# rongzhao-zhang/EfficientQ

Hardware: AMD Instinct MI355X
Metric: ptq_calibration_throughput (higher is better)
Workload: dtype i8xi8->i32 (exact) for the Gram systems and per-iteration loss convs of the layers with quantised input, f32/f64 elsewhere

## Files before the change

### efficientq_amd/_lib.py

```python
from __future__ import annotations

import ctypes as C
import os

import torch

_HERE = os.path.dirname(os.path.abspath(__file__))
LIB_PATH = os.path.join(_HERE, "libeffq_hip.so")

EFFQ_OK = 0
_ERR_NAMES = {1: "EFFQ_ERR_ARG", 2: "EFFQ_ERR_HIP", 3: "EFFQ_ERR_WORKSPACE", 4: "EFFQ_ERR_NO_DEVICE",
              5: "EFFQ_ERR_NOT_CONVERGED"}


class EffqError(RuntimeError):
    pass


class Geom(C.Structure):
    _fields_ = [(n, C.c_int32) for n in
                ("N", "C1", "C2", "D", "H", "W", "KD", "KH", "KW", "SD", "SH", "SW", "PD", "PH", "PW")]

    def out_dims(self):
        return ((self.D + 2 * self.PD - self.KD) // self.SD + 1,
# ... 40 lines not shown


class ProfRecord(C.Structure):
    _fields_ = [("kind", C.c_int32), ("iter", C.c_int32), ("loss_kind", C.c_int32), ("c2", C.c_int32), ("n", C.c_int32),
                ("geom", Geom), ("ms", C.c_float)]


SIGNATURES = {
    "effq_last_error": (C.c_char_p, []),
    "effq_version": (_I, []),
    "effq_device_count": (_I, [C.POINTER(C.c_int)]),
    "effq_quant_dequant_f32": (_I, [_P, _P, _F, _F, _I, _P, _P, _SZ, _P]),
    "effq_quant_dequant_f64path": (_I, [_P, _P, _D, _D, _I, _P, _P, _P, _SZ, _P]),
    "effq_reduce_ws_bytes": (_SZ, []),
    "effq_abs_sum_f64": (_I, [_P, _SZ, _P, _P, _P]),
    "effq_moments_f64": (_I, [_P, _SZ, _P, _P, _P]),
    "effq_alpha_stats_f64": (_I, [_P, _P, _D, _D, _I, _SZ, _P, _P, _P, _P]),
    "effq_fp_init": (_I, [_P, _P, _P]),
    "effq_fp_update": (_I, [_P, _D, _I, _P]),
    "effq_alpha_fixed_point": (_I, [_P, _SZ, _I, _D, _D, _D, _I, _I, _P, _P, _P]),
    "effq_fp_small_max": (_SZ, []),
    "effq_fixed_point_small": (_I, [_P, _P, _P, _SZ, _I, _D, _D, _D, _I, _P, _P]),
    "effq_fp_coop_max": (_SZ, []),
    "effq_fp_coop_set_spin_limit": (_I, [C.c_uint]),
    "effq_fixed_point_coop": (_I, [_P, _P, _P, _SZ, _I, _D, _D, _D, _I, _P, _P, _P]),
    "effq_fp_bucket_max": (_SZ, []),
    "effq_fp_bucket_ws_bytes": (_SZ, [_SZ]),
    "effq_fixed_point_bucket": (_I, [_P, _P, _P, _SZ, _I, _D, _D, _D, _I, _P, _P, _SZ, _P]),
    "effq_fp_bracket_ws_bytes": (_SZ, [_SZ]),
    "effq_fp_bracket_init": (_I, [_P, _P, _SZ, _I, _I, _P, _SZ, _P]),
    "effq_fp_bracket_run": (_I, [_P, _SZ, _I, _D, _D, _D, _I, _I, _P, _P, _P]),
    "effq_fp_bracket_stats": (_I, [_P, _SZ, _I, _D, _D, _P, _P, _P]),
    "effq_fp_bracket_update": (_I, [_SZ, _I, _D, _D, _D, _I, _P, _P, _P]),
    "effq_fp_traj_max": (_SZ, []),
    "effq_fp_traj_ws_bytes": (_SZ, [_SZ]),
    "effq_spd_inverse_prepare": (_I, [_P]),
    "effq_fp_traj_pred_bytes": (_SZ, []),
    "effq_fixed_point_traj": (_I, [_P, _P, _P, _SZ, _I, _D, _D, _D, _I, _P, _P, _P, _SZ, _P]),
    "effq_fixed_point_bucket_rec": (_I, [_P, _P, _P, _SZ, _I, _D, _D, _D, _I, _P, _P, _SZ, _P, _P]),
    "effq_fixed_point_coop_rec": (_I, [_P, _P, _P, _SZ, _I, _D, _D, _D, _I, _P, _P, _P, _P]),
    "effq_fp_check": (_I, [_P, _P, _P]),
    "effq_fp_channels_max_row": (_I, []),
    "effq_fixed_point_channels": (_I, [_P, _P, _P, _I, _I, _I, _D, _I, _P, _P, _P, _P]),
    "effq_fixed_point_channels_proj": (_I, [_P, _P, _P, _I, _I, _I, _D, _I, _P, _P, _P, _P, _F, _P, _P, _P, _I, _I, _D,
                                            _D, _P]),
    "effq_gram_packed_elems": (_SZ, [_I, _I]),
    "effq_gram_pack": (_I, [_P, _P, _I, _I, _P, _P]),
    "effq_gram_unpack": (_I, [_P, _I, _I, _P, _P, _P]),
    "effq_act_quant_backward": (_I, [_P, _P, _I, _P, _P, _P, _SZ, _P, _P]),
    "effq_att_classes_ws_bytes": (_SZ, []),
    "effq_att_classes": (_I, [_P, _LL, _P, _P, _P, C.POINTER(C.c_int32), _P, _P]),
    "effq_prof_enable": (_I, [_I]),
    "effq_prof_count": (_I, []),
    "effq_prof_read": (_I, [_I, C.POINTER(ProfRecord)]),
    "effq_admm_num_inverses": (_I, [_D, _D, _I, _I]),
    "effq_admm_run": (_I, [C.POINTER(AdmmRunArgs)]),
    "effq_admm_select_best": (_I, [_P, _I, _P, _P, _SZ, _SZ, _P, _P, _P, _P]),
    "effq_gram_ws_bytes": (_SZ, [_GP, _I]),
    "effq_gram_accum": (_I, [_P, _P, _P, _GP, _I, _P, _P, _I, _P, _SZ, _P]),
    "effq_gram_plan_query": (_I, [_GP, _I, _IP, _IP, _IP, _IP, _LLP, _IP, _IP]),
    "effq_gram_streamed": (_I, [_P, _P, _GP, _I]),
    "effq_gram_finish": (_I, [_GP, _I, _P, _P, _I, _P, _SZ, _P]),
    "effq_gram_i8_supported": (_I, [_GP, _I]),
    "effq_gram_i8_ws_bytes": (_SZ, [_GP, _I]),
    "effq_gram_accum_i8": (_I, [_P, _P, _GP, _I, _P, _I, _P, _P, _P, _I, _LL, _P, _P, _I, _P, _SZ, _P]),
    "effq_gram_accum_i8_unw": (_I, [_P, _P, _GP, _I, _P, _I, _P, _P, _P, _I, _LL, _P, _P, _I, _P, _P, _P, _SZ, _P]),
# ... 144 lines not shown
```

### efficientq_amd/csrc/fixed_point_bracket.hip

```cpp
#include <math.h>
#include "common.h"
#include "fp_level.h"

namespace effq {

constexpr int FBR_T = 256;
constexpr int FBR_MAXG = 1024;
constexpr int FBR_FT = 1024;
constexpr size_t FBR_MIN_PER = 8192;
enum { FBR_X = 0, FBR_A = 1, FBR_B = 2, FBR_Z = 3 };

struct FbrHdr {
  double blo, bhi;
  double nlo, nhi;
  double alpha_pp;
  double inv_q, q;
  long long src, dst, narrow;
  long long G, per;
  long long escapes, narrowings;
  long long visited;
  long long list_total;
  double r_prev;
  double density;
  long long mono;
  long long planned;
  long long widen;
  long long base;
  long long z_total;
  double guard_lo, guard_hi;
  long long ext[4];
};
static_assert(sizeof(FbrHdr) <= 256, "FbrHdr layout");

struct FbrWs {
  FbrHdr* hdr;
  unsigned* segcnt;
  long long* D;
  long long* U;
  long long* DZ;
  float* L[3];
};
static void fbr_shape(size_t n, size_t* G, size_t* per) {
  size_t g = (n + FBR_MIN_PER - 1) / FBR_MIN_PER;
  if (g < 1) g = 1;
  if (g > (size_t)FBR_MAXG) g = FBR_MAXG;
  size_t p = (n + g - 1) / g;
  p = (p + 3) & ~(size_t)3;
  *G = g;
  *per = p;
}
static size_t fbr_ws_bytes(size_t n) {
  size_t G, per;
  fbr_shape(n, &G, &per);
  return 256 + sizeof(unsigned) * 4 * FBR_MAXG + sizeof(long long) * 12 * FBR_MAXG + 3 * sizeof(float) * (G * per + 64);
}
static FbrWs fbr_carve(void* ws, size_t n) {
  size_t G, per;
  fbr_shape(n, &G, &per);
  FbrWs w;
  char* p = reinterpret_cast<char*>(ws);
  w.hdr = reinterpret_cast<FbrHdr*>(p);
  p += 256;
  w.segcnt = reinterpret_cast<unsigned*>(p);
  p += sizeof(unsigned) * 4 * FBR_MAXG;
  w.D = reinterpret_cast<long long*>(p);
  p += sizeof(long long) * 4 * FBR_MAXG;
  w.U = reinterpret_cast<long long*>(p);
  p += sizeof(long long) * 4 * FBR_MAXG;
  w.DZ = reinterpret_cast<long long*>(p);
  p += sizeof(long long) * 4 * FBR_MAXG;
  for (int i = 0; i < 3; ++i) {
    w.L[i] = reinterpret_cast<float*>(p);
    p += sizeof(float) * (G * per + 64);
  }
  return w;
}

__device__ __forceinline__ long long wave_sum_i64(long long v) {
#pragma unroll
  for (int off = 32; off > 0; off >>= 1) v += __shfl_down(v, off, 64);
  return v;
}

__global__ __launch_bounds__(FBR_T) void k_fbr_iter(const float* __restrict__ x, size_t n, FbrWs w,
                                                    const effq_fp_state* __restrict__ st, double lo, double hi,
                                                    double d, int vec_ok) {
  if (st->done != 0) return;
  __shared__ unsigned s_out;
  __shared__ long long s_red[8][FBR_T / 64];
  const FbrHdr h = *w.hdr;
  const int tid = threadIdx.x, lane = tid & 63, wid = tid >> 6, wg = blockIdx.x;
  const size_t per = (size_t)h.per;
  const float* src;
  size_t cnt;
  if (h.src == FBR_X) {
    const size_t s0 = (size_t)wg * per;
    cnt = (s0 < n) ? ((n - s0 < per) ? n - s0 : per) : 0;
    src = x + s0;
  } else {
    src = w.L[h.src - 1] + (size_t)wg * per;
    cnt = w.segcnt[(h.src - 1) * FBR_MAXG + wg];
  }
  const bool narrow = h.narrow != 0;
  float* __restrict__ dst = w.L[narrow ? h.dst - 1 : 0] + (size_t)wg * per;
  const double aa = st->alpha, al = narrow ? h.nlo : aa, ah = narrow ? h.nhi : aa;
  const LevelConsts la = level_consts(aa, lo, hi, d), ll = level_consts(al, lo, hi, d), lh = level_consts(ah, lo, hi, d);
  const double inv_q = h.inv_q;
  if (tid == 0) s_out = 0u;
  __syncthreads();

  long long D0 = 0, D1 = 0, D2 = 0, D3 = 0, U0 = 0, U1 = 0, U2 = 0, U3 = 0;
  auto tally = [&](float v, bool valid) -> bool {
    const int r = (int)fp_level_f(v, la, aa, lo, hi, d);
    const long long u = __double2ll_rn((double)v * inv_q);
    bool und = true;
    if (narrow) und = (int)fp_level_f(v, ll, al, lo, hi, d) != (int)fp_level_f(v, lh, ah, lo, hi, d);
    const long long ru = (long long)r * u, r1 = valid ? (long long)r : 0ll, r2 = valid ? (long long)(r * r) : 0ll;
    const long long ruv = valid ? ru : 0ll, uv = valid ? u : 0ll;
    if (und) {
      U0 += ruv; U1 += r1; U2 += r2; U3 += uv;
    } else {
      D0 += ruv; D1 += r1; D2 += r2; D3 += uv;
// ... 36 lines not shown
      if (narrow) append4(v, keep);
    }
    if (j0 + FBR_T < nvec_pad) {
      const float v[4] = {qb.x, qb.y, qb.z, qb.w};
      bool keep[4];
#pragma unroll
      for (int c = 0; c < 4; ++c) keep[c] = tally(v[c], vb);
      if (narrow) append4(v, keep);
    }
  }
  const size_t t0 = nvec * 4;
  const size_t ntail_pad = (cnt - t0 + 63) & ~(size_t)63;
  for (size_t j0 = (size_t)wid * 64; j0 < ntail_pad; j0 += FBR_T) {
    const size_t j = t0 + j0 + lane;
    const bool valid = j < cnt;
    const float v[4] = {valid ? src[j] : 0.f, 0.f, 0.f, 0.f};
    bool keep[4] = {tally(v[0], valid), false, false, false};
    if (narrow) append4(v, keep);
  }

  long long acc[8] = {D0, D1, D2, D3, U0, U1, U2, U3};
#pragma unroll
  for (int s = 0; s < 8; ++s) {
    acc[s] = wave_sum_i64(acc[s]);
    if (lane == 0) s_red[s][wid] = acc[s];
  }
  __syncthreads();
  if (tid < 8) {
    long long t = 0;
#pragma unroll
    for (int wv = 0; wv < FBR_T / 64; ++wv) t += s_red[tid][wv];
    if (tid < 4) {
      if (narrow && h.dst == FBR_Z) {
        w.DZ[wg * 4 + tid] = t;
        w.D[wg * 4 + tid] = 0;
      } else if (h.src == FBR_X || h.src == FBR_Z) {
        w.D[wg * 4 + tid] = t;
      } else {
        w.D[wg * 4 + tid] += t;
      }
    } else {
      w.U[wg * 4 + (tid - 4)] = t;
    }
  }
  if (tid == 0 && narrow) w.segcnt[(h.dst - 1) * FBR_MAXG + wg] = s_out;
}

__device__ void fbr_plan(FbrHdr* h, double a_new, double alpha, double a_pp, int it, size_t n) {
  const bool base_z = h->base == FBR_Z;
  if (h->src != FBR_X && !(a_new >= h->blo && a_new <= h->bhi)) {
    h->src = h->base;
    h->blo = fmax(base_z ? 1e-300 : 0.0, h->guard_lo);
    h->bhi = fmin(base_z ? 1e300 : INFINITY, h->guard_hi);
    h->list_total = base_z ? h->z_total : 0;
    h->escapes += 1;
    if (h->planned == 0 && h->widen < 4) h->widen += 1;
    h->planned = 0;
  }
  h->narrow = 0;
  if (!(it >= 2 && a_new > 0.0 && a_new < 1e300)) return;
  const double d1 = a_new - alpha, d0 = alpha - a_pp;
  const double safety = 3.0 * (double)(1 << (int)h->widen);
  const bool at_base = (h->src == h->base);
  double nlo, nhi;
  bool planned = false;
  const double r = d1 / d0;
  if (r > 0.0 && r < 1e6) {
    const double rp = h->r_prev;
    double rc = r;
    if (rp > 0.0 && r > rp) rc = r + 2.0 * (r - rp);
    if (rp > rc) rc = rp;
    if (rc > 0.985) rc = 0.985;
    const double T = d1 * rc / (1.0 - rc);
    const double sg = (T < 0.0) ? -1.0 : 1.0, ad = fabs(d1);
    double ahead = safety * fabs(T) + 0.25 * ad;
    const double behind = (h->mono >= 2) ? 0.1 * ad : 0.5 * fabs(T) + 0.25 * ad;
    if (h->mono >= 2 && ad > 0.0) {
      const double R = base_z ? (double)h->z_total : (double)n;
      const double dens = (h->density > 0.0) ? h->density : R / a_new;
      const double cost_limit = 0.6 * dens * ahead, cost_horizon = 2.0 * sqrt(R * dens * ad);
      if (cost_horizon < 0.8 * cost_limit) {
// ... 4 lines not shown
        planned = true;
      }
    }
    const double fwd = a_new + sg * ahead, back = a_new - sg * behind;
    nlo = fmin(fwd, back);
    nhi = fmax(fwd, back);
    h->r_prev = r;
    h->mono += 1;
  } else {
    const double wdt = safety * fabs(d1);
    nlo = a_new - wdt;
    nhi = a_new + wdt;
    h->r_prev = 0.0;
    h->mono = 0;
  }
  if ((nhi > h->bhi && d1 > 0.0) || (nlo < h->blo && d1 < 0.0)) planned = true;
  nlo = fmax(fmax(nlo, h->blo), a_new * 1e-3);
  nhi = fmin(nhi, h->bhi);
  if (nlo <= a_new && a_new <= nhi && nlo < nhi) {
    const bool worth = at_base || ((nhi - nlo) < 0.7 * (h->bhi - h->blo));
    if (worth) {
      h->narrow = 1;
      h->dst = (h->src == FBR_A) ? FBR_B : FBR_A;
      h->nlo = nlo;
      h->nhi = nhi;
      h->planned = planned ? 1 : 0;
    }
  }
}

__global__ __launch_bounds__(FBR_FT) void k_fbr_finish(FbrWs w, effq_fp_state* st, size_t n, double lo, double d,
                                                      double tol, int max_iter, int mode) {
  if (st->done != 0) return;
  __shared__ long long s_red[5][FBR_FT / 64];
  const int tid = threadIdx.x, lane = tid & 63, wid = tid >> 6;
  FbrHdr* h = w.hdr;
  const int G = (int)h->G;
  if (mode & 1) {
    long long a[5] = {0, 0, 0, 0, 0};
    for (int g = tid; g < G; g += FBR_FT) {
#pragma unroll
      for (int s = 0; s < 4; ++s) a[s] += w.DZ[g * 4 + s] + w.D[g * 4 + s] + w.U[g * 4 + s];
      if (h->narrow != 0) a[4] += (long long)w.segcnt[(h->dst - 1) * FBR_MAXG + g];
    }
#pragma unroll
    for (int s = 0; s < 5; ++s) {
      a[s] = wave_sum_i64(a[s]);
      if (lane == 0) s_red[s][wid] = a[s];
    }
    __syncthreads();
    if (tid == 0) {
      long long t[5];
#pragma unroll
      for (int s = 0; s < 5; ++s) {
        t[s] = (s < 4) ? h->ext[s] : 0;
        for (int wv = 0; wv < FBR_FT / 64; ++wv) t[s] += s_red[s][wv];
      }
      const double q = h->q;
      const double srx = q * (double)t[0], sx = q * (double)t[3];
      st->sums[0] = d * srx + lo * sx;
      st->sums[1] = (d * d * (double)t[2] + 2.0 * d * lo * (double)t[1]) + lo * lo * (double)n;
      h->visited += (h->src == FBR_X) ? (long long)n : h->list_total;
      if (h->narrow != 0) {
        if (h->dst == FBR_Z) {
          h->base = FBR_Z;
          h->z_total = t[4];
        } else if (h->nhi > h->nlo) {
          h->density = (double)t[4] / (h->nhi - h->nlo);
        }
        h->src = h->dst;
        h->blo = h->nlo;
        h->bhi = h->nhi;
        h->list_total = t[4];
        h->narrowings += 1;
        h->narrow = 0;
      }
    }
  }
  if ((mode & 2) && tid == 0) {
    const double alpha = st->alpha;
    const double a_new = st->sums[0] / st->sums[1];
    const double a_pp = st->alpha_prev;
    h->alpha_pp = a_pp;
    st->alpha_prev = alpha;
    st->alpha = a_new;
    const int it = st->iters + 1;
    st->iters = it;
    int done = 0;
    fp_stop(it, max_iter, a_new, alpha, tol, done);
    if (done == 0 && !(a_new >= h->guard_lo && a_new <= h->guard_hi))
      done = 4;
    st->done = done;
    if (done == 0) fbr_plan(h, a_new, alpha, a_pp, it, n);
  }
}

__global__ __launch_bounds__(FBR_T) void k_fbr_init(FbrWs w, effq_fp_state* st, const double* abs_sums, long long G,
                                                    long long per, int levels, int list_first) {
  for (int i = threadIdx.x; i < 4 * FBR_MAXG; i += FBR_T) {
    w.DZ[i] = 0;
    w.D[i] = 0;
    w.U[i] = 0;
  }
  if (threadIdx.x != 0) return;
  const double S = abs_sums[0], cnt = abs_sums[1];
  st->alpha = S / cnt;
  st->alpha_prev = -999.0;
  st->sums[0] = S;
  st->sums[1] = cnt;
  st->iters = 0;
  st->done = 0;
  int e = 0;
  const double bound = (double)(levels - 1) * S;
  if (bound > 0.0 && bound < 1e300) e = 60 - ilogb(bound);
  if (e > 1000) e = 1000;
  if (e < -1000) e = -1000;
  FbrHdr* h = w.hdr;
  h->blo = 0.0;
  h->bhi = INFINITY;
  h->nlo = 0.0;
  h->nhi = INFINITY;
  h->alpha_pp = -999.0;
  h->inv_q = ldexp(1.0, e);
  h->q = ldexp(1.0, -e);
  h->src = FBR_X;
  h->dst = FBR_A;
  h->narrow = list_first ? 1 : 0;
  if (list_first) {
    h->dst = FBR_Z;
    h->nlo = 1e-300;
    h->nhi = 1e300;
  }
  h->G = G;
  h->per = per;
  h->escapes = 0;
  h->narrowings = 0;
  h->visited = 0;
  h->list_total = 0;
  h->r_prev = 0.0;
  h->density = 0.0;
  h->mono = 0;
  h->planned = 0;
  h->widen = 0;
  h->base = FBR_X;
  h->z_total = 0;
  h->guard_lo = 0.0;
  h->guard_hi = INFINITY;
  for (int i = 0; i < 4; ++i) h->ext[i] = 0;
}

__global__ __launch_bounds__(FBR_FT) void k_fbr_export(FbrWs w, long long* __restrict__ out) {
  __shared__ long long s_red[4][FBR_FT / 64];
  const int tid = threadIdx.x, lane = tid & 63, wid = tid >> 6;
  const FbrHdr h = *w.hdr;
  const int G = (int)h.G;
  long long a[4] = {0, 0, 0, 0};
  for (int g = tid; g < G; g += FBR_FT)
#pragma unroll
    for (int s = 0; s < 4; ++s) a[s] += w.DZ[g * 4 + s] + w.D[g * 4 + s];
#pragma unroll
  for (int s = 0; s < 4; ++s) {
    a[s] = wave_sum_i64(a[s]);
    if (lane == 0) s_red[s][wid] = a[s];
  }
  __syncthreads();
  if (tid < 4) {
    long long t = h.ext[tid];
    for (int wv = 0; wv < FBR_FT / 64; ++wv) t += s_red[tid][wv];
    out[tid] = t;
  }
  if (tid == 0) {
    long long run = 0;
    for (int g = 0; g < G; ++g) {
      out[8 + g] = run;
      run += (h.src == FBR_X) ? 0 : (long long)w.segcnt[(h.src - 1) * FBR_MAXG + g];
    }
    out[8 + G] = run;
    out[4] = (h.src == FBR_X) ? -1 : ((h.planned != 0) ? -2 : run);
    out[5] = __double_as_longlong(h.blo);
    out[6] = __double_as_longlong(h.bhi);
  }
// ... 9 lines not shown
  if (ok && h.src != FBR_X) {
    const float* L = w.L[h.src - 1] + (size_t)g * (size_t)h.per;
    const size_t o = (size_t)out[8 + g], c = (size_t)(out[8 + g + 1] - out[8 + g]);
    for (size_t i = tid; i < c; i += FBR_T) list_out[o + i] = L[i];
  }
  const size_t tail = cap - used, per = (tail + G - 1) / G;
  const size_t z0 = used + (size_t)g * per, z1 = (z0 + per < cap) ? z0 + per : cap;
  for (size_t i = z0 + tid; i < z1; i += FBR_T) list_out[i] = 0.0f;
}

__global__ void k_fbr_rebase(FbrWs w, effq_fp_state* st) {
  if (threadIdx.x != 0 || blockIdx.x != 0) return;
  FbrHdr* h = w.hdr;
  const bool base_z = h->base == FBR_Z;
  h->src = h->base;
  h->blo = fmax(base_z ? 1e-300 : 0.0, h->guard_lo);
  h->bhi = fmin(base_z ? 1e300 : INFINITY, h->guard_hi);
  h->list_total = base_z ? h->z_total : 0;
  h->narrow = 0;
  h->planned = 0;
  h->r_prev = 0.0;
  h->mono = 0;
  if (st->done == 4) st->done = 0;
}

__global__ __launch_bounds__(FBR_T) void k_fbr_import(FbrWs dst, const FbrHdr* __restrict__ src_hdr,
                                                      const long long* __restrict__ pack, int world, long long cap,
                                                      long long G, long long per, effq_fp_state* st) {
  for (int i = threadIdx.x; i < 4 * FBR_MAXG; i += FBR_T) {
    dst.DZ[i] = 0;
    dst.D[i] = 0;
    dst.U[i] = 0;
  }
  if (threadIdx.x != 0) return;
  double glo = 0.0, ghi = INFINITY;
  bool ok = st->done == 0;
  for (int r = 0; r < world; ++r) {
    const long long len = pack[4 + 3 * r];
    if (len < 0 || len > cap) ok = false;
    glo = fmax(glo, __longlong_as_double(pack[5 + 3 * r]));
    ghi = fmin(ghi, __longlong_as_double(pack[6 + 3 * r]));
  }
  if (!(glo <= st->alpha && st->alpha <= ghi)) ok = false;
  FbrHdr h = *src_hdr;
  h.guard_lo = glo;
  h.guard_hi = ghi;
  h.blo = glo;
  h.bhi = ghi;
  for (int i = 0; i < 4; ++i) h.ext[i] = pack[i];
  h.r_prev = 0.0;
  h.density = 0.0;
  h.mono = 0;
  h.planned = 0;
  h.widen = 0;
  h.escapes = 0;
  h.narrowings = 0;
  h.visited = 0;
  h.src = FBR_X;
  h.dst = FBR_Z;
  h.narrow = 1;
  h.nlo = fmax(glo, 1e-300);
  h.nhi = fmin(ghi, 1e300);
  h.base = FBR_X;
  h.z_total = 0;
  h.list_total = 0;
  h.G = G;
  h.per = per;
  *dst.hdr = h;
  if (!ok && st->done == 0) st->done = 4;
}

}
using namespace effq;

extern "C" {

size_t effq_fp_bracket_ws_bytes(size_t n) { return fbr_ws_bytes(n); }

int effq_fp_bracket_init(effq_fp_state* state_dev, const double* abs_sums_dev, size_t n, int levels, int list_first,
                         void* ws, size_t ws_bytes, void* stream) {
  EFFQ_CHECK_ARG(state_dev && abs_sums_dev && ws && n > 0 && levels >= 2 && levels <= 256);
  if (ws_bytes < fbr_ws_bytes(n)) {
    set_error("fp_bracket: workspace %zu < %zu bytes", ws_bytes, fbr_ws_bytes(n));
    return EFFQ_ERR_WORKSPACE;
  }
  size_t G, per;
  fbr_shape(n, &G, &per);
  hipLaunchKernelGGL(k_fbr_init, dim3(1), dim3(FBR_T), 0, as_stream(stream), fbr_carve(ws, n), state_dev, abs_sums_dev,
                     (long long)G, (long long)per, levels, list_first);
  EFFQ_LAUNCH_CHECK();
  return EFFQ_OK;
}

static int fbr_launch_iter(const float* x, size_t n, const FbrWs& w, effq_fp_state* st, double lo, double hi, double d,
                           hipStream_t s) {
  size_t G, per;
  fbr_shape(n, &G, &per);
  const int vec_ok = ((reinterpret_cast<uintptr_t>(x) & 15u) == 0) ? 1 : 0;
  hipLaunchKernelGGL(k_fbr_iter, dim3((unsigned)G), dim3(FBR_T), 0, s, x, n, w, st, lo, hi, d, vec_ok);
  return 0;
}

int effq_fp_bracket_run(const float* x, size_t n, int levels, double lo, double hi, double tol, int max_iter, int n_iters,
                        effq_fp_state* state_dev, void* ws, void* stream) {
  EFFQ_CHECK_ARG(x && state_dev && ws && n > 0 && n_iters >= 0 && levels >= 2 && levels <= 256 && hi > lo);
  const double d = (hi - lo) / (double)(levels - 1);
  const FbrWs w = fbr_carve(ws, n);
  hipStream_t s = as_stream(stream);
  for (int i = 0; i < n_iters; ++i) {
    fbr_launch_iter(x, n, w, state_dev, lo, hi, d, s);
    hipLaunchKernelGGL(k_fbr_finish, dim3(1), dim3(FBR_FT), 0, s, w, state_dev, n, lo, d, tol, max_iter, 3);
  }
  EFFQ_LAUNCH_CHECK();
  return EFFQ_OK;
}

int effq_fp_bracket_stats(const float* x, size_t n, int levels, double lo, double hi, effq_fp_state* state_dev, void* ws,
                          void* stream) {
  EFFQ_CHECK_ARG(x && state_dev && ws && n > 0 && levels >= 2 && levels <= 256 && hi > lo);
  const double d = (hi - lo) / (double)(levels - 1);
  const FbrWs w = fbr_carve(ws, n);
  hipStream_t s = as_stream(stream);
  fbr_launch_iter(x, n, w, state_dev, lo, hi, d, s);
  hipLaunchKernelGGL(k_fbr_finish, dim3(1), dim3(FBR_FT), 0, s, w, state_dev, n, lo, d, 0.0, 1, 1);
  EFFQ_LAUNCH_CHECK();
  return EFFQ_OK;
}

size_t effq_fp_bracket_export_words(void) { return 8 + FBR_MAXG + 1; }

int effq_fp_bracket_export(const void* ws, size_t n, long long* out, float* list_out, size_t list_cap, void* stream) {
  EFFQ_CHECK_ARG(ws && out && list_out && n > 0 && list_cap > 0);
  size_t G, per;
  fbr_shape(n, &G, &per);
  const FbrWs w = fbr_carve(const_cast<void*>(ws), n);
  hipLaunchKernelGGL(k_fbr_export, dim3(1), dim3(FBR_FT), 0, as_stream(stream), w, out);
  hipLaunchKernelGGL(k_fbr_export_copy, dim3((unsigned)G), dim3(FBR_T), 0, as_stream(stream), w, out, list_out, list_cap);
  EFFQ_LAUNCH_CHECK();
  return EFFQ_OK;
}

int effq_fp_bracket_import(const void* ws_src, size_t n_src, const long long* pack_dev, int world, size_t list_cap,
                           effq_fp_state* state_dev, void* ws_dst, size_t ws_dst_bytes, void* stream) {
  EFFQ_CHECK_ARG(ws_src && pack_dev && state_dev && ws_dst && n_src > 0 && world > 0 && list_cap > 0 && ws_src != ws_dst);
  const size_t m = (size_t)world * list_cap;
  if (ws_dst_bytes < fbr_ws_bytes(m)) {
    set_error("fp_bracket_import: workspace %zu < %zu bytes", ws_dst_bytes, fbr_ws_bytes(m));
    return EFFQ_ERR_WORKSPACE;
  }
  size_t G, per;
  fbr_shape(m, &G, &per);
  hipLaunchKernelGGL(k_fbr_import, dim3(1), dim3(FBR_T), 0, as_stream(stream), fbr_carve(ws_dst, m),
                     fbr_carve(const_cast<void*>(ws_src), n_src).hdr, pack_dev, world, (long long)list_cap, (long long)G,
                     (long long)per, state_dev);
  EFFQ_LAUNCH_CHECK();
  return EFFQ_OK;
// ... 21 lines not shown
```

### efficientq_amd/hip_ops.py

```python
from __future__ import annotations

import ctypes as C
import math
from typing import Optional, Tuple

import torch

from . import _lib
from ._lib import Geom, check

ADMM_TOL = 1e-5
FP_BRACKET_MIN = 1 << 18
DP_GATHER_AFTER = 4
DP_GATHER_MAX_BYTES = 128 << 20


def _ptr(t: Optional[torch.Tensor]):
    return None if t is None else C.c_void_p(t.data_ptr())


def to_ndhwc(x: torch.Tensor) -> torch.Tensor:
    return x.permute(0, 2, 3, 4, 1).contiguous()


# ... 261 lines not shown
        check(self.lib.effq_fp_bracket_export(_ptr(ws), n, _ptr(exp), _ptr(lst), slot, self.stream),
              "effq_fp_bracket_export")
        pack = torch.zeros(4 + 3 * world, dtype=torch.int64, device=dev)
        pack[:4] = exp[:4]
        pack[4 + 3 * rank: 7 + 3 * rank] = exp[4:7]
        reducer(pack)
        gathered = reducer.all_gather(lst[:slot])
        m = world * slot
        ws2 = self._workspace("fp_bracket_gathered", self.lib.effq_fp_bracket_ws_bytes(m))
        check(self.lib.effq_fp_bracket_import(_ptr(ws), n, _ptr(pack), world, slot, _ptr(st), _ptr(ws2), ws2.numel(),
                                              self.stream), "effq_fp_bracket_import")
        batch = 12 * levels
        while True:
            check(self.lib.effq_fp_bracket_run(_ptr(gathered), m, levels, lo, hi, ADMM_TOL, cap, batch, _ptr(st), _ptr(ws2),
                                               self.stream), "effq_fp_bracket_run")
            alpha, iters, done = self.read_fp_state(st)
            if done == 1:
                return alpha, iters, st
            if done == 2:
                raise RuntimeWarning(f"Exceed maximum iteration ({cap}) for alpha optimization")
            if done == 4:
                check(self.lib.effq_fp_bracket_rebase(_ptr(st), _ptr(ws), n, self.stream), "effq_fp_bracket_rebase")
                lens = pack[4::3].cpu().tolist()
                worst = max(lens) if min(lens) >= 0 else 0
                return DP_GATHER_AFTER if worst <= slot else max(2, min(32, int(math.ceil(3.6 * math.log(worst / slot))) + 1))
            batch = min(2 * batch, 256)

    def fp_bracket_diagnostics(self):
        ws = self._ws["fp_bracket"]
        f = ws[:256].view(torch.float64).cpu()
        i = ws[:256].view(torch.int64).cpu()
        return {"blo": float(f[0]), "bhi": float(f[1]), "src": int(i[7]), "G": int(i[10]), "per": int(i[11]),
                "escapes": int(i[12]), "narrowings": int(i[13]), "visited": int(i[14]), "list_total": int(i[15]),
                "density": float(f[17]), "widen": int(i[20]), "base": int(i[21]), "z_total": int(i[22])}

    def weight_fixed_point(self, wstar, dual, v, levels: int, state, guess: int = 16):
        n = wstar.numel()
        if n <= self.lib.effq_fp_small_max():
            check(self.lib.effq_fixed_point_small(_ptr(wstar), _ptr(dual), _ptr(v), n, levels, -1.0, 1.0, ADMM_TOL,
                                                  100 * levels, _ptr(state), self.stream), "effq_fixed_point_small")
            return None
        if n <= self.lib.effq_fp_coop_max():
            check(self.lib.effq_fixed_point_coop(_ptr(wstar), _ptr(dual), _ptr(v), n, levels, -1.0, 1.0, ADMM_TOL,
                                                 100 * levels, _ptr(state), _ptr(self._red_ws), self.stream),
                  "effq_fixed_point_coop")
            return None
        self.admm_presum(wstar, dual, v)
        _, it, _ = self.fit_scale(v, levels, -1.0, 1.0, guess_iters=guess, state=state)
        return it

    def fixed_point_bucket(self, a, b, v, levels: int, state, lo: float = -1.0, hi: float = 1.0):
        n = a.numel()
        ws = self._workspace("fp_bucket", self.lib.effq_fp_bucket_ws_bytes(n))
        check(self.lib.effq_fixed_point_bucket(_ptr(a), _ptr(b), _ptr(v), n, levels, lo, hi, ADMM_TOL, 100 * levels,
                                               _ptr(state), _ptr(ws), ws.numel(), self.stream),
              "effq_fixed_point_bucket")

    def new_fp_pred(self) -> torch.Tensor:
        return torch.zeros(self.lib.effq_fp_traj_pred_bytes(), dtype=torch.uint8, device=self.device)

    def fixed_point_traj(self, a, b, v, levels: int, state, pred, lo: float = -1.0, hi: float = 1.0):
        n = a.numel()
        ws = self._workspace("fp_traj", self.lib.effq_fp_traj_ws_bytes(n))
        check(self.lib.effq_fixed_point_traj(_ptr(a), _ptr(b), _ptr(v), n, levels, lo, hi, ADMM_TOL, 100 * levels,
                                             _ptr(state), _ptr(pred), _ptr(ws), ws.numel(), self.stream),
              "effq_fixed_point_traj")

# ... 1355 lines not shown
```

### include/effq_hip.h

```cpp
#ifndef EFFQ_HIP_H
#define EFFQ_HIP_H

#include <stddef.h>
#include <stdint.h>

#ifdef __cplusplus
extern "C" {
#endif

enum {
  EFFQ_OK = 0,
  EFFQ_ERR_ARG = 1,
  EFFQ_ERR_HIP = 2,
  EFFQ_ERR_WORKSPACE = 3,
  EFFQ_ERR_NO_DEVICE = 4,
  EFFQ_ERR_NOT_CONVERGED = 5
};

typedef struct effq_geom {
  int32_t N, C1, C2;
  int32_t D, H, W;
  int32_t KD, KH, KW;
  int32_t SD, SH, SW;
  int32_t PD, PH, PW;
// ... 36 lines not shown
int effq_fixed_point_small(const float* a, const float* b, float* v_out, size_t n, int levels, double lo, double hi,
                           double tol, int max_iter, effq_fp_state* state_dev, void* stream);
size_t effq_fp_coop_max(void);
int effq_fixed_point_coop(const float* a, const float* b, float* v_out, size_t n, int levels, double lo, double hi,
                          double tol, int max_iter, effq_fp_state* state_dev, void* ws, void* stream);
int effq_fp_coop_set_spin_limit(unsigned int polls);
size_t effq_fp_bucket_max(void);
size_t effq_fp_bucket_ws_bytes(size_t n);
int effq_fixed_point_bucket(const float* a, const float* b, float* v_out, size_t n, int levels, double lo, double hi,
                            double tol, int max_iter, effq_fp_state* state_dev, void* ws, size_t ws_bytes,
                            void* stream);

size_t effq_fp_traj_max(void);
size_t effq_fp_traj_ws_bytes(size_t n);
size_t effq_fp_traj_pred_bytes(void);
int effq_fixed_point_traj(const float* a, const float* b, float* v_out, size_t n, int levels, double lo, double hi,
                          double tol, int max_iter, effq_fp_state* state_dev, void* pred_dev, void* ws, size_t ws_bytes,
                          void* stream);
int effq_fixed_point_bucket_rec(const float* a, const float* b, float* v_out, size_t n, int levels, double lo, double hi,
                                double tol, int max_iter, effq_fp_state* state_dev, void* ws, size_t ws_bytes,
                                void* pred_dev, void* stream);
int effq_fixed_point_coop_rec(const float* a, const float* b, float* v_out, size_t n, int levels, double lo, double hi,
                              double tol, int max_iter, effq_fp_state* state_dev, void* ws, void* pred_dev, void* stream);

size_t effq_fp_bracket_ws_bytes(size_t n);
int effq_fp_bracket_init(effq_fp_state* state_dev, const double* abs_sums_dev, size_t n, int levels, int list_first,
                         void* ws, size_t ws_bytes, void* stream);
int effq_fp_bracket_run(const float* x, size_t n, int levels, double lo, double hi, double tol, int max_iter, int n_iters,
                        effq_fp_state* state_dev, void* ws, void* stream);
int effq_fp_bracket_stats(const float* x, size_t n, int levels, double lo, double hi, effq_fp_state* state_dev, void* ws,
                          void* stream);
int effq_fp_bracket_update(size_t n, int levels, double lo, double hi, double tol, int max_iter,
                           effq_fp_state* state_dev, void* ws, void* stream);
size_t effq_fp_bracket_export_words(void);
int effq_fp_bracket_export(const void* ws, size_t n, long long* out, float* list_out, size_t list_cap, void* stream);
int effq_fp_bracket_import(const void* ws_src, size_t n_src, const long long* pack_dev, int world, size_t list_cap,
                           effq_fp_state* state_dev, void* ws_dst, size_t ws_dst_bytes, void* stream);
int effq_fp_bracket_rebase(effq_fp_state* state_dev, void* ws, size_t n, void* stream);
int effq_fp_channels_max_row(void);
int effq_fixed_point_channels(const float* a, const float* b, float* v_out, int c2, int nwrow, int levels, double tol,
                              int max_iter, double* alpha_out, int32_t* iters_out, int32_t* err_flag_dev, void* stream);
int effq_fixed_point_channels_proj(const float* wstar, float* dual, float* v_out, int c2, int nwrow, int levels,
                                   double tol, int max_iter, double* alpha_out, int32_t* iters_out, int32_t* err_flag_dev,
                                   float* G, float dual_div, float* Bm, const float* B0, const float* W0, int n, int ldb,
                                   double rho_next, double eta, void* stream);

int effq_fp_check(const effq_fp_state* state_dev, int32_t* err_flag_dev, void* stream);

size_t effq_gram_ws_bytes(const effq_geom* g, int has_bias);
int effq_gram_accum(const float* x_ndhwc, const float* att, const float* y_ndhwc, const effq_geom* g,
                    int has_bias, float* A0, float* B0, int accumulate, void* ws, size_t ws_bytes,
                    void* stream);
int effq_gram_plan_query(const effq_geom* g, int has_bias, int* vec, int* nb, int* npairs, int* nsplit,
                         long long* vox_per_split, int* fold, int* finish_blocks);
int effq_gram_streamed(const float* x_ndhwc, const float* y_ndhwc, const effq_geom* g, int has_bias);
int effq_gram_finish(const effq_geom* g, int has_bias, float* A0, float* B0, int accumulate, void* ws, size_t ws_bytes,
                     void* stream);

int effq_gram_i8_supported(const effq_geom* g, int act_levels);
size_t effq_gram_i8_ws_bytes(const effq_geom* g, int ncls);
int effq_gram_accum_i8(const uint8_t* xidx_ndhwc, const float* y_ndhwc, const effq_geom* g, int has_bias,
                       const float* act_alpha_dev, int act_levels, const int32_t* vox_list,
                       const int32_t* chunk_cls, const float* cls_w_dev, int ncls, long long n_list,
                       float* A0, float* B0, int accumulate, void* ws, size_t ws_bytes, void* stream);
int effq_gram_accum_i8_unw(const uint8_t* xidx_ndhwc, const float* y_ndhwc, const effq_geom* g, int has_bias,
                           const float* act_alpha_dev, int act_levels, const int32_t* vox_list, const int32_t* chunk_cls,
// ... 272 lines not shown
```

Measured before the change: 25.46.

## Fuse bracket fixed-point finish into iteration kernel via last-block ticket and LDS tail loop

Each bracket iteration used to launch the per-block tally kernel and then a separate single-block finish kernel. Now the last block to arrive, detected through grouped atomic tickets, does the reduction, commit, update and planning itself, which removes one launch per iteration. When the active candidate list is small, that block also keeps iterating on the list in LDS inside the same launch, so further iterations need no relaunch at all. The cost is a large shared-memory footprint (an 8K-float cache plus prefix arrays) that may lower occupancy of the main pass, extra atomics, and subtle memory-ordering risks.

```diff
diff --git a/efficientq_amd/_lib.py b/efficientq_amd/_lib.py
--- a/efficientq_amd/_lib.py
+++ b/efficientq_amd/_lib.py
@@ -96,6 +96,7 @@
     "effq_fp_bracket_run": (_I, [_P, _SZ, _I, _D, _D, _D, _I, _I, _P, _P, _P]),
     "effq_fp_bracket_stats": (_I, [_P, _SZ, _I, _D, _D, _P, _P, _P]),
     "effq_fp_bracket_update": (_I, [_SZ, _I, _D, _D, _D, _I, _P, _P, _P]),
+    "effq_fp_bracket_set_tail": (_I, [_SZ]),
     "effq_fp_traj_max": (_SZ, []),
     "effq_fp_traj_ws_bytes": (_SZ, [_SZ]),
     "effq_spd_inverse_prepare": (_I, [_P]),
diff --git a/efficientq_amd/csrc/fixed_point_bracket.hip b/efficientq_amd/csrc/fixed_point_bracket.hip
--- a/efficientq_amd/csrc/fixed_point_bracket.hip
+++ b/efficientq_amd/csrc/fixed_point_bracket.hip
@@ -1,4 +1,5 @@
 #include <math.h>
+#include <stddef.h>
 #include "common.h"
 #include "fp_level.h"
 
@@ -29,8 +30,14 @@
   long long z_total;
   double guard_lo, guard_hi;
   long long ext[4];
+  unsigned ticket, pad;
+  long long passes;
 };
-static_assert(sizeof(FbrHdr) <= 256, "FbrHdr layout");
+static_assert(sizeof(FbrHdr) <= 256 && offsetof(FbrHdr, ext) == 200 && offsetof(FbrHdr, passes) == 240, "FbrHdr layout");
+
+constexpr int FBR_TAIL_LDS = 8192;
+constexpr size_t FBR_TAIL_MAX = 8192;
+static size_t g_fbr_tail_max = FBR_TAIL_MAX;
 
 struct FbrWs {
   FbrHdr* hdr;
@@ -76,18 +83,210 @@
   return w;
 }
 
+template <class V>
+__device__ __forceinline__ void fbr_publish(V* p, V v) {
+  __hip_atomic_store(p, v, __ATOMIC_RELAXED, __HIP_MEMORY_SCOPE_AGENT);
+}
+
 __device__ __forceinline__ long long wave_sum_i64(long long v) {
 #pragma unroll
   for (int off = 32; off > 0; off >>= 1) v += __shfl_down(v, off, 64);
   return v;
 }
 
-__global__ __launch_bounds__(FBR_T) void k_fbr_iter(const float* __restrict__ x, size_t n, FbrWs w,
-                                                    const effq_fp_state* __restrict__ st, double lo, double hi,
-                                                    double d, int vec_ok) {
-  if (st->done != 0) return;
-  __shared__ unsigned s_out;
-  __shared__ long long s_red[8][FBR_T / 64];
+__device__ void fbr_plan(FbrHdr* h, double a_new, double alpha, double a_pp, int it, size_t n);
+
+template <int T>
+__device__ __forceinline__ void fbr_sum_tallies(const FbrWs& w, const FbrHdr* h, long long (*s_red)[T / 64],
+                                                long long (&t)[9]) {
+  const int tid = threadIdx.x, lane = tid & 63, wid = tid >> 6;
+  const int G = (int)h->G;
+  const bool narrow = h->narrow != 0;
+  const unsigned* cnt = w.segcnt + (narrow ? h->dst - 1 : 0) * FBR_MAXG;
+  long long a[9] = {0, 0, 0, 0, 0, 0, 0, 0, 0};
+  for (int g = tid; g < G; g += T) {
+#pragma unroll
+    for (int s = 0; s < 4; ++s) {
+      a[s] += w.DZ[g * 4 + s] + w.D[g * 4 + s];
+      a[4 + s] += w.U[g * 4 + s];
+    }
+    if (narrow) a[8] += (long long)cnt[g];
+  }
+#pragma unroll
+  for (int s = 0; s < 9; ++s) {
+    a[s] = wave_sum_i64(a[s]);
+    if (lane == 0) s_red[s][wid] = a[s];
+  }
+  __syncthreads();
+  if (tid == 0) {
+#pragma unroll
+    for (int s = 0; s < 9; ++s) {
+      t[s] = (s < 4) ? h->ext[s] : 0;
+      for (int wv = 0; wv < T / 64; ++wv) t[s] += s_red[s][wv];
+    }
+  }
+}
+
+__device__ __forceinline__ void fbr_store_sums(const FbrHdr* h, effq_fp_state* st, const long long (&t)[4], size_t n,
+                                               double lo, double d) {
+#pragma clang fp contract(off)
+  const double q = h->q;
+  const double srx = q * (double)t[0], sx = q * (double)t[3];
+  st->sums[0] = d * srx + lo * sx;
+  st->sums[1] = (d * d * (double)t[2] + 2.0 * d * lo * (double)t[1]) + lo * lo * (double)n;
+}
+
+__device__ __forceinline__ void fbr_commit(FbrHdr* h, effq_fp_state* st, const long long (&t)[9], size_t n, double lo,
+                                           double d) {
+  const long long all[4] = {t[0] + t[4], t[1] + t[5], t[2] + t[6], t[3] + t[7]};
+  fbr_store_sums(h, st, all, n, lo, d);
+  h->visited += (h->src == FBR_X) ? (long long)n : h->list_total;
+  h->passes += 1;
+  if (h->narrow != 0) {
+    if (h->dst == FBR_Z) {
+      h->base = FBR_Z;
+      h->z_total = t[8];
+    } else if (h->nhi > h->nlo) {
+      h->density = (double)t[8] / (h->nhi - h->nlo);
+    }
+    h->src = h->dst;
+    h->blo = h->nlo;
+    h->bhi = h->nhi;
+    h->list_total = t[8];
+    h->narrowings += 1;
+    h->narrow = 0;
+  }
+}
+
+__device__ __forceinline__ int fbr_update(FbrHdr* h, effq_fp_state* st, double tol, int max_iter) {
+#pragma clang fp contract(off)
+  const double alpha = st->alpha;
+  const double a_new = st->sums[0] / st->sums[1];
+  h->alpha_pp = st->alpha_prev;
+  st->alpha_prev = alpha;
+  st->alpha = a_new;
+  const int it = st->iters + 1;
+  st->iters = it;
+  int done = 0;
+  fp_stop(it, max_iter, a_new, alpha, tol, done);
+  if (done == 0 && !(a_new >= h->guard_lo && a_new <= h->guard_hi))
+    done = 4;
+  st->done = done;
+  return done;
+}
+
+struct FbrLast {
+  FbrHdr h;
+  effq_fp_state st;
+  float v[FBR_TAIL_LDS];
+  unsigned pre[FBR_MAXG + 1];
+  unsigned wtot[FBR_T / 64];
+  int last, go;
+};
+static_assert(FBR_MAXG == 4 * FBR_T, "fbr_tail: four segments per thread");
+
+__device__ __forceinline__ int fbr_tail_next(FbrHdr* h, long long kind, size_t tail_max) {
+  const long long src = h->src;
+  if ((src != FBR_A && src != FBR_B) || tail_max == 0 || (size_t)h->list_total > tail_max) return 0;
+  if (h->narrow != 0) {
+    if (h->list_total > (long long)FBR_TAIL_LDS) return 0;
+    h->narrow = 0;
+    h->planned = kind;
+  }
+  return 1;
+}
+
+__device__ __forceinline__ void fbr_tail(const FbrWs& w, FbrLast& sm, long long (*s_red)[FBR_T / 64],
+                                         const long long (&dec)[4], size_t n, double lo, double hi, double d, double tol,
+                                         int max_iter, size_t tail_max) {
+  const int tid = threadIdx.x, lane = tid & 63, wid = tid >> 6;
+  const int src = (int)sm.h.src, G = (int)sm.h.G;
+  const size_t per = (size_t)sm.h.per;
+  const double inv_q = sm.h.inv_q;
+  const unsigned* cnt = w.segcnt + (src - 1) * FBR_MAXG;
+  const float* L = w.L[src - 1];
+  unsigned c[4], loc = 0u;
+#pragma unroll
+  for (int k = 0; k < 4; ++k) {
+    const int g = tid * 4 + k;
+    c[k] = (g < G) ? cnt[g] : 0u;
+    loc += c[k];
+  }
+  unsigned inc = loc;
+#pragma unroll
+  for (int off = 1; off < 64; off <<= 1) {
+    const unsigned o = __shfl_up(inc, off, 64);
+    if (lane >= off) inc += o;
+  }
+  if (lane == 63) sm.wtot[wid] = inc;
+  __syncthreads();
+  unsigned run = inc - loc;
+  for (int wv = 0; wv < wid; ++wv) run += sm.wtot[wv];
+#pragma unroll
+  for (int k = 0; k < 4; ++k) {
+    sm.pre[tid * 4 + k] = run;
+    run += c[k];
+  }
+  if (tid == FBR_T - 1) sm.pre[FBR_MAXG] = run;
+  __syncthreads();
+  const unsigned total = sm.pre[FBR_MAXG];
+  auto fetch = [&](unsigned i) -> float {
+    int a = 0, b = FBR_MAXG;
+    while (b - a > 1) {
+      const int m = (a + b) >> 1;
+      if (sm.pre[m] <= i) a = m; else b = m;
+    }
+    return L[(size_t)a * per + (i - sm.pre[a])];
+  };
+  const bool cached = total <= (unsigned)FBR_TAIL_LDS;
+  if (cached) {
+    for (unsigned i = tid; i < total; i += FBR_T) sm.v[i] = fetch(i);
+    __syncthreads();
+  }
+  for (;;) {
+    const double aa = sm.st.alpha;
+    const LevelConsts la = level_consts(aa, lo, hi, d);
+    long long a[4] = {0, 0, 0, 0};
+    for (unsigned i = tid; i < total; i += FBR_T) {
+      const float v = cached ? sm.v[i] : fetch(i);
+      const int r = (int)fp_level_f(v, la, aa, lo, hi, d);
+      const long long u = __double2ll_rn((double)v * inv_q);
+      a[0] += (long long)r * u;
+      a[1] += (long long)r;
+      a[2] += (long long)(r * r);
+      a[3] += u;
+    }
+#pragma unroll
+    for (int s = 0; s < 4; ++s) {
+      a[s] = wave_sum_i64(a[s]);
+      if (lane == 0) s_red[s][wid] = a[s];
+    }
+    __syncthreads();
+    if (tid == 0) {
+      long long t[4];
+#pragma unroll
+      for (int s = 0; s < 4; ++s) {
+        t[s] = dec[s];
+        for (int wv = 0; wv < FBR_T / 64; ++wv) t[s] += s_red[s][wv];
+      }
+      fbr_store_sums(&sm.h, &sm.st, t, n, lo, d);
+      sm.h.visited += sm.h.list_total;
+      int go = 0;
+      if (fbr_update(&sm.h, &sm.st, tol, max_iter) == 0) {
+        const long long kind = sm.h.planned;
+        fbr_plan(&sm.h, sm.st.alpha, sm.st.alpha_prev, sm.h.alpha_pp, sm.st.iters, n);
+        go = fbr_tail_next(&sm.h, kind, tail_max);
+      }
+      sm.go = go;
+    }
+    __syncthreads();
+    if (sm.go == 0) break;
+  }
+}
+
+__device__ __forceinline__ void fbr_pass(const float* __restrict__ x, size_t n, const FbrWs& w, const effq_fp_state* st,
+                                         double lo, double hi, double d, int vec_ok, unsigned& s_out,
+                                         long long (*s_red)[FBR_T / 64]) {
   const FbrHdr h = *w.hdr;
   const int tid = threadIdx.x, lane = tid & 63, wid = tid >> 6, wg = blockIdx.x;
   const size_t per = (size_t)h.per;
@@ -190,21 +389,85 @@
     for (int wv = 0; wv < FBR_T / 64; ++wv) t += s_red[tid][wv];
     if (tid < 4) {
       if (narrow && h.dst == FBR_Z) {
-        w.DZ[wg * 4 + tid] = t;
-        w.D[wg * 4 + tid] = 0;
+        fbr_publish(&w.DZ[wg * 4 + tid], t);
+        fbr_publish(&w.D[wg * 4 + tid], 0ll);
       } else if (h.src == FBR_X || h.src == FBR_Z) {
-        w.D[wg * 4 + tid] = t;
+        fbr_publish(&w.D[wg * 4 + tid], t);
       } else {
-        w.D[wg * 4 + tid] += t;
+        fbr_publish(&w.D[wg * 4 + tid], w.D[wg * 4 + tid] + t);
       }
     } else {
-      w.U[wg * 4 + (tid - 4)] = t;
-    }
-  }
-  if (tid == 0 && narrow) w.segcnt[(h.dst - 1) * FBR_MAXG + wg] = s_out;
-}
-
-__device__ void fbr_plan(FbrHdr* h, double a_new, double alpha, double a_pp, int it, size_t n) {
+      fbr_publish(&w.U[wg * 4 + (tid - 4)], t);
+    }
+  }
+  if (tid == 0 && narrow) fbr_publish(&w.segcnt[(h.dst - 1) * FBR_MAXG + wg], s_out);
+}
+
+__global__ __launch_bounds__(FBR_T) void k_fbr_iter(const float* __restrict__ x, size_t n, FbrWs w, effq_fp_state* st,
+                                                    double lo, double hi, double d, int vec_ok, int fuse, double tol,
+                                                    int max_iter, size_t tail_max) {
+  if (st->done != 0) return;
+  __shared__ unsigned s_out;
+  __shared__ long long s_red[9][FBR_T / 64];
+  __shared__ FbrLast sm;
+  fbr_pass(x, n, w, st, lo, hi, d, vec_ok, s_out, s_red);
+  if (fuse == 0) return;
+  const int tid = threadIdx.x;
+  asm volatile("s_waitcnt vmcnt(0)" ::: "memory");
+  __syncthreads();
+  if (tid == 0) {
+    const unsigned G = gridDim.x, grp = blockIdx.x >> 5, ngrp = (G + 31u) >> 5;
+    const unsigned gsize = (grp + 1u < ngrp) ? 32u : G - grp * 32u;
+    unsigned* gt = w.segcnt + 3 * FBR_MAXG + grp * 32u;
+    int last = 0;
+    if (__hip_atomic_fetch_add(gt, 1u, __ATOMIC_RELAXED, __HIP_MEMORY_SCOPE_AGENT) == gsize - 1u) {
+      __hip_atomic_store(gt, 0u, __ATOMIC_RELAXED, __HIP_MEMORY_SCOPE_AGENT);
+      last = __hip_atomic_fetch_add(&w.hdr->ticket, 1u, __ATOMIC_RELAXED, __HIP_MEMORY_SCOPE_AGENT) == ngrp - 1u;
+    }
+    sm.last = last;
+  }
+  __syncthreads();
+  if (!sm.last) return;
+  if (tid == 0) {
+    __builtin_amdgcn_fence(__ATOMIC_ACQUIRE, "agent");
+    asm volatile("s_waitcnt vmcnt(0)" ::: "memory");
+  }
+  __syncthreads();
+  unsigned long long* gh = reinterpret_cast<unsigned long long*>(w.hdr);
+  unsigned long long* gs = reinterpret_cast<unsigned long long*>(st);
+  unsigned long long* sh = reinterpret_cast<unsigned long long*>(&sm.h);
+  unsigned long long* ss = reinterpret_cast<unsigned long long*>(&sm.st);
+  constexpr int HW = sizeof(FbrHdr) / 8, SW = sizeof(effq_fp_state) / 8;
+  static_assert(sizeof(FbrHdr) % 8 == 0 && sizeof(effq_fp_state) % 8 == 0 && HW <= 64 && SW <= 64, "one word per thread");
+  if (tid < HW) sh[tid] = gh[tid];
+  if (tid >= 64 && tid < 64 + SW) ss[tid - 64] = gs[tid - 64];
+  __syncthreads();
+  long long t[9];
+  fbr_sum_tallies<FBR_T>(w, &sm.h, s_red, t);
+  if (tid == 0) {
+    const bool narrowed = sm.h.narrow != 0;
+    fbr_commit(&sm.h, &sm.st, t, n, lo, d);
+    int go = 0;
+    if (fbr_update(&sm.h, &sm.st, tol, max_iter) == 0) {
+      const long long kind = sm.h.planned;
+      fbr_plan(&sm.h, sm.st.alpha, sm.st.alpha_prev, sm.h.alpha_pp, sm.st.iters, n);
+      go = fbr_tail_next(&sm.h, kind, tail_max);
+      if (narrowed) go = 0;
+    }
+    sm.go = go;
+  }
+  __syncthreads();
+  if (sm.go != 0) {
+    const long long dec[4] = {t[0], t[1], t[2], t[3]};
+    fbr_tail(w, sm, s_red, dec, n, lo, hi, d, tol, max_iter, tail_max);
+  }
+  if (tid == 0) sm.h.ticket = 0u;
+  __syncthreads();
+  if (tid < HW) gh[tid] = sh[tid];
+  if (tid >= 64 && tid < 64 + SW) gs[tid - 64] = ss[tid - 64];
+}
+
+__device__ __attribute__((noinline)) void fbr_plan(FbrHdr* h, double a_new, double alpha, double a_pp, int it, size_t n) {
   const bool base_z = h->base == FBR_Z;
   if (h->src != FBR_X && !(a_new >= h->blo && a_new <= h->bhi)) {
     h->src = h->base;
@@ -275,66 +538,15 @@
 __global__ __launch_bounds__(FBR_FT) void k_fbr_finish(FbrWs w, effq_fp_state* st, size_t n, double lo, double d,
                                                       double tol, int max_iter, int mode) {
   if (st->done != 0) return;
-  __shared__ long long s_red[5][FBR_FT / 64];
-  const int tid = threadIdx.x, lane = tid & 63, wid = tid >> 6;
+  __shared__ long long s_red[9][FBR_FT / 64];
   FbrHdr* h = w.hdr;
-  const int G = (int)h->G;
   if (mode & 1) {
-    long long a[5] = {0, 0, 0, 0, 0};
-    for (int g = tid; g < G; g += FBR_FT) {
-#pragma unroll
-      for (int s = 0; s < 4; ++s) a[s] += w.DZ[g * 4 + s] + w.D[g * 4 + s] + w.U[g * 4 + s];
-      if (h->narrow != 0) a[4] += (long long)w.segcnt[(h->dst - 1) * FBR_MAXG + g];
-    }
-#pragma unroll
-    for (int s = 0; s < 5; ++s) {
-      a[s] = wave_sum_i64(a[s]);
-      if (lane == 0) s_red[s][wid] = a[s];
-    }
-    __syncthreads();
-    if (tid == 0) {
-      long long t[5];
-#pragma unroll
-      for (int s = 0; s < 5; ++s) {
-        t[s] = (s < 4) ? h->ext[s] : 0;
-        for (int wv = 0; wv < FBR_FT / 64; ++wv) t[s] += s_red[s][wv];
-      }
-      const double q = h->q;
-      const double srx = q * (double)t[0], sx = q * (double)t[3];
-      st->sums[0] = d * srx + lo * sx;
-      st->sums[1] = (d * d * (double)t[2] + 2.0 * d * lo * (double)t[1]) + lo * lo * (double)n;
-      h->visited += (h->src == FBR_X) ? (long long)n : h->list_total;
-      if (h->narrow != 0) {
-        if (h->dst == FBR_Z) {
-          h->base = FBR_Z;
-          h->z_total = t[4];
-        } else if (h->nhi > h->nlo) {
-          h->density = (double)t[4] / (h->nhi - h->nlo);
-        }
-        h->src = h->dst;
-        h->blo = h->nlo;
-        h->bhi = h->nhi;
-        h->list_total = t[4];
-        h->narrowings += 1;
-        h->narrow = 0;
-      }
-    }
-  }
-  if ((mode & 2) && tid == 0) {
-    const double alpha = st->alpha;
-    const double a_new = st->sums[0] / st->sums[1];
-    const double a_pp = st->alpha_prev;
-    h->alpha_pp = a_pp;
-    st->alpha_prev = alpha;
-    st->alpha = a_new;
-    const int it = st->iters + 1;
-    st->iters = it;
-    int done = 0;
-    fp_stop(it, max_iter, a_new, alpha, tol, done);
-    if (done == 0 && !(a_new >= h->guard_lo && a_new <= h->guard_hi))
-      done = 4;
-    st->done = done;
-    if (done == 0) fbr_plan(h, a_new, alpha, a_pp, it, n);
+    long long t[9];
+    fbr_sum_tallies<FBR_FT>(w, h, s_red, t);
+    if (threadIdx.x == 0) fbr_commit(h, st, t, n, lo, d);
+  }
+  if ((mode & 2) && threadIdx.x == 0) {
+    if (fbr_update(h, st, tol, max_iter) == 0) fbr_plan(h, st->alpha, st->alpha_prev, h->alpha_pp, st->iters, n);
   }
 }
 
@@ -345,6 +557,7 @@
     w.D[i] = 0;
     w.U[i] = 0;
   }
+  for (int i = threadIdx.x; i < FBR_MAXG; i += FBR_T) w.segcnt[3 * FBR_MAXG + i] = 0u;
   if (threadIdx.x != 0) return;
   const double S = abs_sums[0], cnt = abs_sums[1];
   st->alpha = S / cnt;
@@ -390,6 +603,9 @@
   h->guard_lo = 0.0;
   h->guard_hi = INFINITY;
   for (int i = 0; i < 4; ++i) h->ext[i] = 0;
+  h->ticket = 0u;
+  h->pad = 0u;
+  h->passes = 0;
 }
 
 __global__ __launch_bounds__(FBR_FT) void k_fbr_export(FbrWs w, long long* __restrict__ out) {
@@ -465,6 +681,7 @@
     dst.D[i] = 0;
     dst.U[i] = 0;
   }
+  for (int i = threadIdx.x; i < FBR_MAXG; i += FBR_T) dst.segcnt[3 * FBR_MAXG + i] = 0u;
   if (threadIdx.x != 0) return;
   double glo = 0.0, ghi = INFINITY;
   bool ok = st->done == 0;
@@ -499,6 +716,8 @@
   h.list_total = 0;
   h.G = G;
   h.per = per;
+  h.ticket = 0u;
+  h.passes = 0;
   *dst.hdr = h;
   if (!ok && st->done == 0) st->done = 4;
 }
@@ -526,12 +745,18 @@
 }
 
 static int fbr_launch_iter(const float* x, size_t n, const FbrWs& w, effq_fp_state* st, double lo, double hi, double d,
-                           hipStream_t s) {
+                           int fuse, double tol, int max_iter, hipStream_t s) {
   size_t G, per;
   fbr_shape(n, &G, &per);
   const int vec_ok = ((reinterpret_cast<uintptr_t>(x) & 15u) == 0) ? 1 : 0;
-  hipLaunchKernelGGL(k_fbr_iter, dim3((unsigned)G), dim3(FBR_T), 0, s, x, n, w, st, lo, hi, d, vec_ok);
+  hipLaunchKernelGGL(k_fbr_iter, dim3((unsigned)G), dim3(FBR_T), 0, s, x, n, w, st, lo, hi, d, vec_ok, fuse, tol,
+                     max_iter, g_fbr_tail_max);
   return 0;
+}
+
+int effq_fp_bracket_set_tail(size_t max_values) {
+  g_fbr_tail_max = (max_values == (size_t)-1) ? FBR_TAIL_MAX : max_values;
+  return EFFQ_OK;
 }
 
 int effq_fp_bracket_run(const float* x, size_t n, int levels, double lo, double hi, double tol, int max_iter, int n_iters,
@@ -540,10 +765,7 @@
   const double d = (hi - lo) / (double)(levels - 1);
   const FbrWs w = fbr_carve(ws, n);
   hipStream_t s = as_stream(stream);
-  for (int i = 0; i < n_iters; ++i) {
-    fbr_launch_iter(x, n, w, state_dev, lo, hi, d, s);
-    hipLaunchKernelGGL(k_fbr_finish, dim3(1), dim3(FBR_FT), 0, s, w, state_dev, n, lo, d, tol, max_iter, 3);
-  }
+  for (int i = 0; i < n_iters; ++i) fbr_launch_iter(x, n, w, state_dev, lo, hi, d, 1, tol, max_iter, s);
   EFFQ_LAUNCH_CHECK();
   return EFFQ_OK;
 }
@@ -554,7 +776,7 @@
   const double d = (hi - lo) / (double)(levels - 1);
   const FbrWs w = fbr_carve(ws, n);
   hipStream_t s = as_stream(stream);
-  fbr_launch_iter(x, n, w, state_dev, lo, hi, d, s);
+  fbr_launch_iter(x, n, w, state_dev, lo, hi, d, 0, 0.0, 1, s);
   hipLaunchKernelGGL(k_fbr_finish, dim3(1), dim3(FBR_FT), 0, s, w, state_dev, n, lo, d, 0.0, 1, 1);
   EFFQ_LAUNCH_CHECK();
   return EFFQ_OK;
diff --git a/efficientq_amd/hip_ops.py b/efficientq_amd/hip_ops.py
--- a/efficientq_amd/hip_ops.py
+++ b/efficientq_amd/hip_ops.py
@@ -317,7 +317,8 @@
         i = ws[:256].view(torch.int64).cpu()
         return {"blo": float(f[0]), "bhi": float(f[1]), "src": int(i[7]), "G": int(i[10]), "per": int(i[11]),
                 "escapes": int(i[12]), "narrowings": int(i[13]), "visited": int(i[14]), "list_total": int(i[15]),
-                "density": float(f[17]), "widen": int(i[20]), "base": int(i[21]), "z_total": int(i[22])}
+                "density": float(f[17]), "widen": int(i[20]), "base": int(i[21]), "z_total": int(i[22]),
+                "passes": int(i[30])}
 
     def weight_fixed_point(self, wstar, dual, v, levels: int, state, guess: int = 16):
         n = wstar.numel()
diff --git a/include/effq_hip.h b/include/effq_hip.h
--- a/include/effq_hip.h
+++ b/include/effq_hip.h
@@ -92,6 +92,7 @@
                           void* stream);
 int effq_fp_bracket_update(size_t n, int levels, double lo, double hi, double tol, int max_iter,
                            effq_fp_state* state_dev, void* ws, void* stream);
+int effq_fp_bracket_set_tail(size_t max_values);
 size_t effq_fp_bracket_export_words(void);
 int effq_fp_bracket_export(const void* ws, size_t n, long long* out, float* list_out, size_t list_cap, void* stream);
 int effq_fp_bracket_import(const void* ws_src, size_t n_src, const long long* pack_dev, int world, size_t list_cap,
```

After: 25.45. About the same (-0.0%).
